# gyoge0/sub_volume_renderer

Hardware: AMD Instinct MI355X
Metric: Mray-steps/sec (+ frames/sec) of the LMIP sub-volume march at 1920x1080, 3-LOD 1024^3 volume (higher is better)
Workload: dtype f32

## Files before the change

sub_volume_renderer_amd/csrc/march_kernel.hip:

```cpp
#include <stdlib.h>

#include <algorithm>
#include <type_traits>

#include "svr_internal.h"

namespace {

struct f3 { float x, y, z; };
struct f4 { float x, y, z, w; };

__device__ __forceinline__ f4 mat_vec(const float* m, float x, float y, float z, float w) {
    f4 r;
    r.x = ((m[0] * x + m[4] * y) + m[8]  * z) + m[12] * w;
    r.y = ((m[1] * x + m[5] * y) + m[9]  * z) + m[13] * w;
    r.z = ((m[2] * x + m[6] * y) + m[10] * z) + m[14] * w;
    r.w = ((m[3] * x + m[7] * y) + m[11] * z) + m[15] * w;
    return r;
}

__device__ __forceinline__ float dot3(f3 a, f3 b) { return (a.x * b.x + a.y * b.y) + a.z * b.z; }

__device__ __forceinline__ uint32_t wrap(uint32_t t, uint32_t wrap0, uint32_t ring) {
    uint32_t w = t + wrap0;
// ... 348 lines not shown
__device__ __forceinline__ float texel_value(float t) { return t; }
__device__ __forceinline__ float texel_value(uint32_t t) { return (float)t; }
__device__ __forceinline__ float texel_abs(float t) { return fabsf(t); }
__device__ __forceinline__ uint32_t texel_abs(uint32_t t) { return t; }
__device__ __forceinline__ float texel_max(float a, float b) { return fmaxf(a, b); }
__device__ __forceinline__ uint32_t texel_max(uint32_t a, uint32_t b) { return max(a, b); }

template <int ESH>
__device__ __forceinline__ typename Texel<ESH>::type lds_texel(uint32_t a) {
#if defined(__HIP_DEVICE_COMPILE__)
    typedef __attribute__((address_space(3))) const uint8_t* p8_t;
    typedef __attribute__((address_space(3))) const uint16_t* p16_t;
    typedef __attribute__((address_space(3))) const float* p32_t;
    if constexpr (ESH == 2) return *(p32_t)a;
    else if constexpr (ESH == 1) return (uint32_t)*(p16_t)a;
    else return (uint32_t)*(p8_t)a;
#else
    (void)a;
    return typename Texel<ESH>::type();
#endif
}

template <int ESH>
__device__ __forceinline__ typename Texel<ESH>::type fetch_density(__amdgpu_buffer_rsrc_t rsrc, uint32_t off, uint32_t soff = 0u) {
    if constexpr (ESH == 2) return __builtin_bit_cast(float, __builtin_amdgcn_raw_buffer_load_b32(rsrc, (int)off, (int)soff, 0));
    else if constexpr (ESH == 1) return (uint32_t)(uint16_t)__builtin_amdgcn_raw_buffer_load_b16(rsrc, (int)off, (int)soff, 0);
    else return (uint32_t)(uint8_t)__builtin_amdgcn_raw_buffer_load_b8(rsrc, (int)off, (int)soff, 0);
}

__device__ __forceinline__ uint32_t mad24(uint32_t a, uint32_t b, uint32_t c) {
    uint32_t r;
    asm("v_mad_u32_u24 %0, %1, %2, %3" : "=v"(r) : "v"(a), "v"(b), "v"(c));
    return r;
}
template <int SH>
__device__ __forceinline__ uint32_t shl_add_c(uint32_t a, uint32_t c) {
    if (SH == 0) return a + c;
    uint32_t r;
    asm("v_lshl_add_u32 %0, %1, %2, %3" : "=v"(r) : "v"(a), "n"(SH), "v"(c));
    return r;
}

template <int ESH> struct TwinBlock { static constexpr int XB = ESH == 0 ? 3 : 2, YB = 2, ZB = ESH == 2 ? 1 : 2; };
struct TwinConsts { uint32_t row_w, inb_w, nbx32; };
template <int ESH>
__device__ __forceinline__ TwinConsts twin_consts(uint32_t Rx, uint32_t Ry) {
    typedef TwinBlock<ESH> B;
    TwinConsts c;
    c.row_w = 1u | (((Ry >> B::YB) * (4u >> B::ZB)) << 16);
    c.inb_w = (1u << (B::XB + ESH)) | ((1u << (B::XB + B::YB + ESH)) << 16);
    c.nbx32 = (Rx >> B::XB) * 32u;
    return c;
}
typedef unsigned short ushort2_t __attribute__((ext_vector_type(2)));
template <int ESH>
__device__ __forceinline__ uint32_t twin_offset_packed(uint32_t x, uint32_t yz, const TwinConsts& c, uint32_t KbS) {
    typedef TwinBlock<ESH> B;
    constexpr uint32_t xm = (1u << B::XB) - 1u, zm = (1u << B::ZB) - 1u, low = 3u | (zm << 16);
    const uint32_t xin = ESH == 0 ? ((x & xm) | KbS) : (((x & xm) << ESH) | KbS);
    const uint32_t inb = __builtin_amdgcn_udot2(__builtin_bit_cast(ushort2_t, yz & low), __builtin_bit_cast(ushort2_t, c.inb_w), xin, false);
    const uint32_t row4 = __builtin_amdgcn_udot2(__builtin_bit_cast(ushort2_t, yz & ~low), __builtin_bit_cast(ushort2_t, c.row_w), 0u, false);
    return __umul24(row4, c.nbx32) + (((x & ~xm) << (7 - B::XB)) + inb);
}
typedef short short2_t __attribute__((ext_vector_type(2)));
typedef float float2_t __attribute__((ext_vector_type(2)));

template <bool SC>
__device__ __forceinline__ float2_t coord_pair(float2_t iter, float s, float t, float ss) {
    if constexpr (SC) return iter * t + s;
    else return (iter * t + s) * ss;
}
template <bool SC>
__device__ __forceinline__ float coord_one(float iter, float s, float t, float ss) {
    if constexpr (SC) return iter * t + s;
    else return (iter * t + s) * ss;
}

struct Idx2 { uint32_t x0, y0, z0, x1, y1, z1; };
template <bool SC>
__device__ __forceinline__ Idx2 voxel_pair(float sx, float sy, float sz, float tx, float ty, float tz, float2_t iter,
                                           float ssx, float ssy, float ssz) {
    const float2_t cx = coord_pair<SC>(iter, sx, tx, ssx);
    const float2_t cy = coord_pair<SC>(iter, sy, ty, ssy);
    const float2_t cz = coord_pair<SC>(iter, sz, tz, ssz);
    Idx2 r;
    r.x0 = (uint32_t)(int)cx.x; r.x1 = (uint32_t)(int)cx.y;
    r.y0 = (uint32_t)(int)cy.x; r.y1 = (uint32_t)(int)cy.y;
    r.z0 = (uint32_t)(int)cz.x; r.z1 = (uint32_t)(int)cz.y;
    return r;
}

struct Idx2p { uint32_t x0, yz0, x1, yz1; };
template <bool SC>
__device__ __forceinline__ Idx2p voxel_pair_packed(float sx, float sy, float sz, float tx, float ty, float tz, float2_t iter,
                                                   float ssx, float ssy, float ssz) {
    const float2_t cx = coord_pair<SC>(iter, sx, tx, ssx);
    const float2_t cy = coord_pair<SC>(iter, sy, ty, ssy);
    const float2_t cz = coord_pair<SC>(iter, sz, tz, ssz);
    Idx2p r;
    r.x0 = (uint32_t)(int)cx.x; r.x1 = (uint32_t)(int)cx.y;
    r.yz0 = (uint32_t)(int)cy.x; r.yz1 = (uint32_t)(int)cy.y;
    asm("v_cvt_i32_f32_sdwa %0, %1 dst_sel:WORD_1 dst_unused:UNUSED_PRESERVE src0_sel:DWORD" : "+v"(r.yz0) : "v"(cz.x));
    asm("v_cvt_i32_f32_sdwa %0, %1 dst_sel:WORD_1 dst_unused:UNUSED_PRESERVE src0_sel:DWORD" : "+v"(r.yz1) : "v"(cz.y));
    return r;
}
__device__ __forceinline__ uint32_t dot2_u16(uint32_t a, uint32_t b, uint32_t c) {
    uint32_t r;
    asm("v_dot2_u32_u16 %0, %1, %2, %3" : "=v"(r) : "v"(a), "s"(b), "v"(c));
    return r;
}
template <typename T> __device__ __forceinline__ T undefined_value() { T v; asm volatile("" : "=v"(v)); return v; }

__device__ __forceinline__ void wave_min3_max3(int& a, int& b, int& c, int& d, int& e, int& f) {
#define SVR_STEP6(ctrl)                              \
    "v_min_i32_dpp %0, %0, %0 " ctrl "\n"            \
    "v_min_i32_dpp %1, %1, %1 " ctrl "\n"            \
    "v_min_i32_dpp %2, %2, %2 " ctrl "\n"            \
    "v_max_i32_dpp %3, %3, %3 " ctrl "\n"            \
    "v_max_i32_dpp %4, %4, %4 " ctrl "\n"            \
    "v_max_i32_dpp %5, %5, %5 " ctrl "\n"
    asm volatile("s_nop 1\n"
                 SVR_STEP6("quad_perm:[1,0,3,2] row_mask:0xf bank_mask:0xf")
                 SVR_STEP6("quad_perm:[2,3,0,1] row_mask:0xf bank_mask:0xf")
                 SVR_STEP6("row_half_mirror row_mask:0xf bank_mask:0xf")
                 SVR_STEP6("row_mirror row_mask:0xf bank_mask:0xf")
                 SVR_STEP6("row_bcast:15 row_mask:0xa bank_mask:0xf")
                 SVR_STEP6("row_bcast:31 row_mask:0xc bank_mask:0xf")
                 "s_nop 0"
                 : "+v"(a), "+v"(b), "+v"(c), "+v"(d), "+v"(e), "+v"(f));
#undef SVR_STEP6
    a = __builtin_amdgcn_readlane(a, 63); b = __builtin_amdgcn_readlane(b, 63); c = __builtin_amdgcn_readlane(c, 63);
    d = __builtin_amdgcn_readlane(d, 63); e = __builtin_amdgcn_readlane(e, 63); f = __builtin_amdgcn_readlane(f, 63);
}

template <bool MAX>
__device__ __forceinline__ int wave_reduce(int v) {
#define SVR_STEP1(ctrl) "s_nop 1\n" "v_min_i32_dpp %0, %0, %0 " ctrl "\n"
#define SVR_STEP1X(ctrl) "s_nop 1\n" "v_max_i32_dpp %0, %0, %0 " ctrl "\n"
    if (MAX)
        asm volatile(SVR_STEP1X("quad_perm:[1,0,3,2] row_mask:0xf bank_mask:0xf")
                     SVR_STEP1X("quad_perm:[2,3,0,1] row_mask:0xf bank_mask:0xf")
                     SVR_STEP1X("row_half_mirror row_mask:0xf bank_mask:0xf")
                     SVR_STEP1X("row_mirror row_mask:0xf bank_mask:0xf")
                     SVR_STEP1X("row_bcast:15 row_mask:0xa bank_mask:0xf")
                     SVR_STEP1X("row_bcast:31 row_mask:0xc bank_mask:0xf")
                     "s_nop 0" : "+v"(v));
    else
        asm volatile(SVR_STEP1("quad_perm:[1,0,3,2] row_mask:0xf bank_mask:0xf")
                     SVR_STEP1("quad_perm:[2,3,0,1] row_mask:0xf bank_mask:0xf")
                     SVR_STEP1("row_half_mirror row_mask:0xf bank_mask:0xf")
                     SVR_STEP1("row_mirror row_mask:0xf bank_mask:0xf")
                     SVR_STEP1("row_bcast:15 row_mask:0xa bank_mask:0xf")
                     SVR_STEP1("row_bcast:31 row_mask:0xc bank_mask:0xf")
                     "s_nop 0" : "+v"(v));
#undef SVR_STEP1
#undef SVR_STEP1X
    return __builtin_amdgcn_readlane(v, 63);
}

struct LodK {
    uint32_t ring[3];
    float    scale[3];
    int32_t  addw[3];
    uint32_t rx4, base_bytes;
    float    ss[3];
    int32_t  slab;
    const void* rbase;
    uint32_t rbytes;
    uint32_t nparts, zsplit, part_bytes, rbytes_last;
    uint32_t twin;
};
__device__ __forceinline__ LodK load_lod(kparams_t p, int l) {
    LodK k;
#pragma unroll
    for (int a = 0; a < 3; ++a) {
        k.ring[a] = p->lod[l].ring[a]; k.scale[a] = p->lod[l].scale[a]; k.addw[a] = p->lod[l].addw[a]; k.ss[a] = p->lod[l].ss[a];
    }
    k.rx4 = p->lod[l].rx4; k.base_bytes = p->lod[l].base_bytes; k.slab = p->lod[l].slab;
    k.rbase = p->lod[l].rbase; k.rbytes = p->lod[l].rbytes;
    k.nparts = p->lod[l].nparts; k.zsplit = p->lod[l].zsplit; k.part_bytes = p->lod[l].part_bytes; k.rbytes_last = p->lod[l].rbytes_last;
    k.twin = p->lod[l].twin;
    return k;
}

struct LodEvents {
    int a, b;
    int cx, cy, cz;
};


template <int NL, int U, bool COUNT, int ESH, bool BIG, bool WAVG = false, bool SCALED = false>
__global__ __launch_bounds__(256) __attribute__((amdgpu_waves_per_eu(SCALED && !COUNT ? 5 : 1))) void march_span(const MarchParams P) {
    static_assert(!(SCALED && WAVG), "the weighted-average reducer reads the unscaled step");
    extern __shared__ __attribute__((aligned(16))) uint8_t lds_all[];
    const int nblocks = P.tiles_x * P.tiles_y;
    const int tb = P.tile_order ? (int)P.tile_order[blockIdx.x] : xcd_remap((int)blockIdx.x, nblocks);
    const int tile_x = tb % P.tiles_x, tile_y = tb / P.tiles_x;
    const int wave = __builtin_amdgcn_readfirstlane((int)(threadIdx.x >> 6)), lane = threadIdx.x & 63;
    const int lw = P.tile_log2w, wl = P.block_waves_log2;
    const int c0 = ((tile_x << wl) + (wave & wl)) << lw, r0 = ((tile_y << wl) + (wave >> 1)) << (6 - lw);
    int lc = lane & ((1 << lw) - 1), lr = lane >> lw;
    {
        const float pcx = (float)(P.frame.x0 + c0) + 0.5f * (float)(1 << lw);
        const float pcy = (float)(P.frame.y0 + (r0 / P.frame.band_h) * P.frame.band_pitch + (r0 % P.frame.band_h)) +
                          0.5f * (float)(64 >> lw);
        const float ncx = 2.0f * pcx / (float)P.frame.frame_w - 1.0f;
        const float ncy = 1.0f - 2.0f * pcy / (float)P.frame.frame_h;
        const float dx = (P.xdir[0] - ncx * P.xdir[3]) * (float)P.frame.frame_w;
        const float dy = (P.xdir[1] - ncy * P.xdir[3]) * (float)P.frame.frame_h;
        if (P.orient && fabsf(dy) > fabsf(dx)) { lr = lane & ((64 >> lw) - 1); lc = lane >> (6 - lw); }
    }
    const int c = c0 + lc;
    const int r = r0 + lr;
    const bool inside = c < P.frame.out_w && r < P.frame.out_h;
    const size_t o = (size_t)r * (size_t)P.frame.out_w + (size_t)c;
    const int x = P.frame.x0 + c;
    const int y = P.frame.y0 + (r / P.frame.band_h) * P.frame.band_pitch + (r % P.frame.band_h);

    unsigned long long t_acc[16] = { 0, 0, 0, 0, 0, 0, 0, 0, 0, 0, 0, 0, 0, 0, 0, 0 };
    unsigned long long t_last = COUNT ? __builtin_amdgcn_s_memtime() : 0ull;
    auto lap = [&](int k) {
        if (COUNT) {
            const unsigned long long t = __builtin_amdgcn_s_memtime();
            t_acc[k] += t - t_last;
            t_last = t;
        }
    };

    Ray Rs;
    Rs.nsteps = 0; Rs.start = { 0.f, 0.f, 0.f }; Rs.step = { 0.f, 0.f, 0.f };
    const bool frag = inside && (x < P.frame.frame_w && y < P.frame.frame_h) && setup_ray(P, x, y, Rs);
    const int nsteps = frag ? Rs.nsteps : 0;
    float Rsx = frag ? Rs.start.x : 0.f, Rsy = frag ? Rs.start.y : 0.f, Rsz = frag ? Rs.start.z : 0.f;
    float Rtx = frag ? Rs.step.x : 0.f, Rty = frag ? Rs.step.y : 0.f, Rtz = frag ? Rs.step.z : 0.f;

    float d0[3], d1[3];
    {
        const float lastf = (float)(nsteps - 1);
        d0[0] = (Rsx + 0.0f * Rtx) * P.size[0];  d1[0] = (Rsx + lastf * Rtx) * P.size[0];
        d0[1] = (Rsy + 0.0f * Rty) * P.size[1];  d1[1] = (Rsy + lastf * Rty) * P.size[1];
        d0[2] = (Rsz + 0.0f * Rtz) * P.size[2];  d1[2] = (Rsz + lastf * Rtz) * P.size[2];
    }
    LodEvents ev[NL];
#pragma unroll
    for (int l = 0; l < NL; ++l) {
        const LodParams& L = P.lod[l];
        int a = 0, b = nsteps, cr[3] = { 0, 0, 0 };
        if (L.shape[0] == 0 || L.shape[1] == 0 || L.shape[2] == 0) {
            ev[l].a = 0; ev[l].b = 0; ev[l].cx = 0; ev[l].cy = 0; ev[l].cz = 0;
            continue;
        }
#pragma unroll
        for (int ax = 0; ax < 3; ++ax) {
            const float st = ax == 0 ? Rsx : (ax == 1 ? Rsy : Rsz);
            const float sp = ax == 0 ? Rtx : (ax == 1 ? Rty : Rtz);
            const bool inc = sp > 0.0f;
            const int v0 = (int)(d0[ax] * L.scale[ax]), v1 = (int)(d1[ax] * L.scale[ax]);
            auto cross = [&](int T) {
                const bool p0 = inc ? v0 >= T : v0 < T;
                const bool p1 = inc ? v1 >= T : v1 < T;
                int j = p0 ? 0 : nsteps;
                const bool need = !p0 && p1;
                if (__builtin_amdgcn_ballot_w64(need) != 0) {
                    const int js = first_cross(nsteps, st, sp, P.size[ax], L.scale[ax], T, need);
                    j = need ? js : j;
                }
                return j;
            };
            const int lo = L.off[ax], hi = L.off[ax] + (int)L.shape[ax];
            const int jlo = cross(lo);
            const int jhi = cross(hi);
            int en = inc ? jlo : jhi, ex = inc ? jhi : jlo;
            if (!(sp > 0.0f) && !(sp < 0.0f)) {
                en = 0; ex = (lo <= v0 && v0 < hi) ? nsteps : 0;
            }
            a = max(a, en); b = min(b, ex);
            if (L.wrap0[ax] + L.shape[ax] > L.ring[ax])
                cr[ax] = cross((int)L.ring[ax] - L.addw[ax]);
            else
                cr[ax] = inc ? nsteps : 0;
        }
        if (a >= b || L.shape[0] == 0) { a = 0; b = 0; }
        ev[l].a = a; ev[l].b = b; ev[l].cx = cr[0]; ev[l].cy = cr[1]; ev[l].cz = cr[2];
    }

    __amdgpu_buffer_rsrc_t rsrc_all = __builtin_amdgcn_make_buffer_rsrc(
        const_cast<void*>(P.density_all), 0, (int)P.density_all_bytes, 0x00020000);

#ifdef SVR_EXPERIMENTS
    const int dbg_nowait = P.dbg_nowait, brick_pow2 = P.brick_pow2;
#else
    constexpr int dbg_nowait = 0, brick_pow2 = 0;
#endif
    bool found = false, finished = (dbg_nowait & 2) != 0;
    float local_max = 0.f, samp = 0.f;
    int hit_i = 0, since = 0;
    uint32_t steps = 0;

    typedef typename Texel<ESH>::type texel_t;
    texel_t thr_raw;
    if constexpr (ESH != 2) thr_raw = P.lmip_threshold_raw; else thr_raw = P.lmip_threshold;
    const bool mip_like = (P.skip_flags & 2) != 0;
    float den = 0.f;
    auto lmip_batch = [&](const texel_t (&sv)[U], int nb, bool live, bool tail) {
        if constexpr (WAVG) {
            const float steplen = sqrtf((Rtx * Rtx + Rty * Rty) + Rtz * Rtz);
            const float k = fresh_params(P)->weight_falloff;
#pragma unroll
            for (int u = 0; u < U; ++u) {
                const bool act = live && !finished && (!tail || (nb + u) < nsteps);
                const float tw = 1.0f - k * ((float)(nb + u) * steplen);
                const bool go = act && tw > 0.0f;
                finished = finished || (act && !go);
                if (COUNT) steps += go ? 1u : 0u;
                const float val = texel_value(sv[u]);
                const float w = tw * tw;
                const float contribution = w * fabsf(val);
                const float num1 = samp + w * val, den1 = den + w;
                samp = go ? num1 : samp;
                den = go ? den1 : den;
                const bool take = go && contribution > local_max;
                local_max = take ? contribution : local_max;
                hit_i = take ? (nb + u) : hit_i;
            }
            return;
        }
        texel_t m;
        if constexpr (ESH != 2) m = 0u; else m = -1.0f;
        const texel_t neutral = m;
#pragma unroll
        for (int u = 0; u < U; ++u) m = texel_max(m, (tail && (nb + u) >= nsteps) ? neutral : texel_abs(sv[u]));
        bool need;
        if (mip_like) need = live && (found ? texel_value(m) > local_max : m >= thr_raw);
        else need = live && (found || m >= thr_raw);
        if (__builtin_amdgcn_ballot_w64(need) != 0) {
#pragma unroll
            for (int u = 0; u < U; ++u) {
                const bool act = live && !finished && (!tail || (nb + u) < nsteps);
                const float val = texel_value(sv[u]);
                const float inten = fabsf(val);
                if (COUNT) steps += act ? 1u : 0u;
                const bool was_found = found;
                const bool first_hit = act && !was_found && inten >= P.lmip_threshold;
                const bool tracking = act && was_found;
                since += tracking ? 1 : 0;
                const bool take = first_hit || (tracking && inten > local_max);
                local_max = take ? inten : local_max;
                samp = take ? val : samp;
                hit_i = take ? (nb + u) : hit_i;
                found = found || first_hit;
                const bool brk = tracking && (since >= P.lmip_max_samples || inten < local_max * P.lmip_fall_off);
                finished = finished || brk;
            }
        } else if (COUNT) {
            steps += live ? (uint32_t)(tail ? (min(nb + U, nsteps) - nb) : U) : 0u;
        }
    };

    int code = NL, E = 0;
    uint32_t Kc = 0xFFFFFFFFu;
    uint32_t Kb = 0u;
    int zth = 0;

    int brick_mode = 0;
    bool many_lines = false;
    if (P.brick) {
        const float pf = (float)min(max(nsteps - 1, 0), 256);
        const int qx = (int)((Rsx + pf * Rtx) * P.size[0]) >> (7 - ESH);
        const int qy = (int)((Rsy + pf * Rty) * P.size[1]);
        const int qz = (int)((Rsz + pf * Rtz) * P.size[2]);
        const int key = frag ? ((qz * 4099 + qy) * 64 + (qx & 63)) : -1 - lane;
        const int k0 = __builtin_amdgcn_update_dpp(key, key, 0x00, 0xF, 0xF, false);
        const int k1 = __builtin_amdgcn_update_dpp(key, key, 0x55, 0xF, 0xF, false);
        const int k2 = __builtin_amdgcn_update_dpp(key, key, 0xAA, 0xF, 0xF, false);
        const int q = lane & 3;
        const bool fresh = frag && (q == 0 || (key != k0 && (q == 1 || (key != k1 && (q == 2 || key != k2)))));
        const int lines = __builtin_popcountll(__builtin_amdgcn_ballot_w64(fresh));
        const int quads = __builtin_popcountll(__builtin_amdgcn_ballot_w64(frag && q == 0)) + 1;
        const bool use_brick = P.brick >= 2 || lines * 16 > P.brick_lines * quads;
        brick_mode = use_brick ? 1 + P.slab_long : 0;
        many_lines = use_brick;
    }
    const int wave_lds = wave * P.brick_bytes;

    int c_general = 0, c_direct = 0, c_brick = 0, c_slabs = 0, c_runs = 0, c_zero = 0, c_skip = 0;
    int n = 0;
    lap(0);
    while (true) {
        const bool alive = !finished && n < nsteps;
        const unsigned long long alive_mask = __builtin_amdgcn_ballot_w64(alive);
        if (alive_mask == 0) break;

        if (__builtin_amdgcn_ballot_w64(alive && n >= E) != 0) {
            const kparams_t Pr = fresh_params(P);
            if (alive && n >= E) {
                code = NL; E = nsteps; Kc = 0xFFFFFFFFu;
                bool settled = false;
#pragma unroll
                for (int l = 0; l < NL; ++l) {
                    const bool in = !settled && n >= ev[l].a && n < ev[l].b;
                    if (in) {
                        const LodK L = load_lod(Pr, l);
                        code = l;
                        E = min(E, ev[l].b);
                        const bool px = (n >= ev[l].cx) == (Rtx > 0.0f);
                        const bool py = (n >= ev[l].cy) == (Rty > 0.0f);
                        const bool pz = (n >= ev[l].cz) == (Rtz > 0.0f);
                        const uint32_t kx = (uint32_t)L.addw[0] - (px ? L.ring[0] : 0u);
                        const uint32_t ky = (uint32_t)L.addw[1] - (py ? L.ring[1] : 0u);
                        const uint32_t kz = (uint32_t)L.addw[2] - (pz ? L.ring[2] : 0u);
                        Kc = (kz * L.ring[1] + ky) * L.rx4 + (kx << ESH) + L.base_bytes;
                        if (many_lines && L.twin) {
                            typedef TwinBlock<ESH> B;
                            Kb = (uint32_t)(((int)kz >> B::ZB) * (int)(L.ring[1] >> B::YB) + ((int)ky >> B::YB)) * (L.ring[0] >> B::XB) +
                                 (uint32_t)((int)kx >> B::XB);
                        }
                        if constexpr (BIG) zth = (int)L.zsplit - (int)kz;
                        if (ev[l].cx > n) E = min(E, ev[l].cx);
                        if (ev[l].cy > n) E = min(E, ev[l].cy);
                        if (ev[l].cz > n) E = min(E, ev[l].cz);
                    } else if (!settled && ev[l].a > n) {
                        E = min(E, ev[l].a);
                    }
                    settled = settled || in;
                }
            }
        }

        const int first = __builtin_amdgcn_readlane(code, (int)__builtin_ctzll(alive_mask));
        int lane_run = (code == first) ? ((E == nsteps ? E - n + U - 1 : E - n) / U) : 0;
        if (first < NL && !fresh_params(P)->lod_pow2[first < NL ? first : 0]) lane_run = alive ? 0 : lane_run;
        if (!alive) lane_run = 0x3fffffff;
        int run = wave_reduce<false>(lane_run);
        if (COUNT) ++c_runs;
        lap(1);

        if (run <= 0) {
            if (COUNT) ++c_general;
            const kparams_t Pg = fresh_params(P);
            texel_t s[U];
            const float basef = (float)n;
            if constexpr (!BIG) {
                uint32_t off[U];
#pragma unroll
                for (int u = 0; u < U; ++u) {
                    off[u] = 0xFFFFFFFFu;
                    const float iter = basef + (float)u;
                    const float dx = (Rsx + iter * Rtx) * Pg->size[0];
                    const float dy = (Rsy + iter * Rty) * Pg->size[1];
                    const float dz = (Rsz + iter * Rtz) * Pg->size[2];
                    bool done = !alive || (n + u) >= nsteps;
#pragma unroll
                    for (int l = 0; l < NL; ++l) {
                        const bool sel = !done && (n + u) >= ev[l].a && (n + u) < ev[l].b;
                        if (__builtin_amdgcn_ballot_w64(sel) != 0) {
                            const uint32_t ofs = lod_offset_wrapped<ESH>(load_lod(Pg, l), dx, dy, dz);
                            off[u] = sel ? ofs : off[u];
                        }
                        done = done || sel;
                    }
                }
#pragma unroll
                for (int u = 0; u < U; ++u) s[u] = fetch_density<ESH>(rsrc_all, off[u]);
            } else {
#pragma unroll
                for (int u = 0; u < U; ++u) {
                    const float iter = basef + (float)u;
                    const float dx = (Rsx + iter * Rtx) * Pg->size[0];
                    const float dy = (Rsy + iter * Rty) * Pg->size[1];
                    const float dz = (Rsz + iter * Rtz) * Pg->size[2];
                    bool done = !alive || (n + u) >= nsteps;
                    texel_t acc = 0;
#pragma unroll
                    for (int l = 0; l < NL; ++l) {
                        const bool sel = !done && (n + u) >= ev[l].a && (n + u) < ev[l].b;
                        if (__builtin_amdgcn_ballot_w64(sel) != 0) {
                            const LodK Lg = load_lod(Pg, l);
                            uint32_t part;
                            const uint32_t ofs = lod_offset_wrapped_split<ESH>(Lg, dx, dy, dz, part);
                            for (unsigned long long todo = __builtin_amdgcn_ballot_w64(sel); todo != 0ull;) {
                                const uint32_t p = (uint32_t)__builtin_amdgcn_readlane((int)part, (int)__builtin_ctzll(todo));
                                const bool mine = sel && part == p;
                                const texel_t t = fetch_density<ESH>(part_rsrc(Lg, p), mine ? ofs : 0xFFFFFFFFu);
                                acc = mine ? t : acc;
                                todo &= ~__builtin_amdgcn_ballot_w64(mine);
                            }
                        }
                        done = done || sel;
                    }
                    s[u] = acc;
                }
            }
            lmip_batch(s, n, alive, true);
            n += U;
            lap(2);
            continue;
        }

        if (first == NL) {
            texel_t s[U];
#pragma unroll
            for (int u = 0; u < U; ++u) s[u] = 0;
            for (; run > 0; --run) {
                if (COUNT) ++c_zero;
                const bool lv = alive && !finished && n < nsteps;
                if (__builtin_amdgcn_ballot_w64(lv && n + U > nsteps) != 0) lmip_batch(s, n, lv, true);
                else lmip_batch(s, n, lv, false);
                n += U;
                if (__builtin_amdgcn_ballot_w64(alive && !finished && n < nsteps) == 0) break;
            }
            continue;
        }

        {
            const LodK L = load_lod(fresh_params(P), first);
            const float ssx = L.ss[0], ssy = L.ss[1], ssz = L.ss[2];
            if constexpr (SCALED) { Rsx *= ssx; Rsy *= ssy; Rsz *= ssz; Rtx *= ssx; Rty *= ssy; Rtz *= ssz; }
            __amdgpu_buffer_rsrc_t rsrc = rsrc_all;
            if constexpr (BIG) rsrc = __builtin_amdgcn_make_buffer_rsrc(const_cast<void*>(L.rbase), 0, (int)L.rbytes, 0x00020000);
            const bool ring_split = BIG && L.nparts > 1u;
            const bool use_twin = many_lines && L.twin == 1u;

            int held = 0;
            do {
            run += held; held = 0;
            if (P.cells_all_bytes != 0u) {
                const kparams_t Ps = fresh_params(P);
                const int sb = Ps->lod[first].skip_batches;
                if (sb > 0 && run >= 4 * sb) {
                    const float reach = (float)(8 * sb);
                    const uint32_t cs = (uint32_t)Ps->lod[first].cshift;
                    const float vx = SCALED ? Rtx : Rtx * ssx, vy = SCALED ? Rty : Rty * ssy, vz = SCALED ? Rtz : Rtz * ssz;
                    const bool slow = fmaxf(fmaxf(fabsf(vx), fabsf(vy)), fabsf(vz)) * reach <=
                                      (float)(1u << cs) - 0.5f;
                    __amdgpu_buffer_rsrc_t crsrc = __builtin_amdgcn_make_buffer_rsrc(
                        const_cast<void*>(Ps->cells_all), 0, (int)Ps->cells_all_bytes, 0x00020000);
                    const uint32_t cbase = Ps->lod[first].cell_base;
                    const uint32_t cdx = Ps->lod[first].cdim[0], cdy = Ps->lod[first].cdim[1], cdz = Ps->lod[first].cdim[2];
                    bool vetoed = false, tracking_only = false;
                    uint32_t c0x, c0y, c0z;
                    {
                        const float i0 = fminf((float)n, (float)(nsteps - 1));
                        c0x = ((uint32_t)(int)coord_one<SCALED>(i0, Rsx, Rtx, ssx) + (uint32_t)L.addw[0]) >> cs;
                        c0y = ((uint32_t)(int)coord_one<SCALED>(i0, Rsy, Rty, ssy) + (uint32_t)L.addw[1]) >> cs;
                        c0z = ((uint32_t)(int)coord_one<SCALED>(i0, Rsz, Rtz, ssz) + (uint32_t)L.addw[2]) >> cs;
                    }
                    while (run >= 4 * sb) {
                        const bool live = alive && !finished && n < nsteps;
                        const float lastf = fminf((float)(nsteps - 1), (float)n + 4.0f * reach - (run > 4 * sb ? 0.0f : 1.0f));
                        uint32_t px[5], py[5], pz[5];
                        px[0] = c0x; py[0] = c0y; pz[0] = c0z;
#pragma unroll
                        for (int g = 1; g < 5; g += 2) {
                            const float i0 = (float)n + reach * (float)g;
                            const float2_t iter = { fminf(i0, lastf), fminf(i0 + reach, lastf) };
                            const Idx2 q = voxel_pair<SCALED>(Rsx, Rsy, Rsz, Rtx, Rty, Rtz, iter, ssx, ssy, ssz);
                            px[g] = (q.x0 + (uint32_t)L.addw[0]) >> cs; py[g] = (q.y0 + (uint32_t)L.addw[1]) >> cs; pz[g] = (q.z0 + (uint32_t)L.addw[2]) >> cs;
                            px[g + 1] = (q.x1 + (uint32_t)L.addw[0]) >> cs; py[g + 1] = (q.y1 + (uint32_t)L.addw[1]) >> cs;
                            pz[g + 1] = (q.z1 + (uint32_t)L.addw[2]) >> cs;
                        }
                        c0x = px[4]; c0y = py[4]; c0z = pz[4];
                        texel_t v[4];
#pragma unroll
                        for (int g = 0; g < 4; ++g) {
                            uint32_t bx = min(px[g], px[g + 1]), by = min(py[g], py[g + 1]), bz = min(pz[g], pz[g + 1]);
                            bx = min(bx, bx - cdx); by = min(by, by - cdy); bz = min(bz, bz - cdz);
                            v[g] = fetch_density<ESH>(crsrc, (__umul24(__umul24(bz, cdy) + by, cdx) + bx) << ESH, cbase);
                        }
                        const texel_t m = texel_max(texel_max(texel_abs(v[0]), texel_abs(v[1])), texel_max(texel_abs(v[2]), texel_abs(v[3])));
                        const bool occupied = live && !found && (!slow || m >= thr_raw);
                        const bool following = live && found && (!mip_like || !slow || texel_value(m) > local_max);
                        const unsigned long long occ_mask = __builtin_amdgcn_ballot_w64(occupied);
                        if (occ_mask != 0 || __builtin_amdgcn_ballot_w64(following) != 0) {
                            vetoed = true;
                            tracking_only = occ_mask == 0;
                            break;
                        }
                        if (COUNT) { steps += live ? (uint32_t)(min(n + 32 * sb, nsteps) - n) : 0u; c_skip += 4 * sb; }
                        n += 32 * sb;
                        run -= 4 * sb;
                        if (__builtin_amdgcn_ballot_w64(alive && !finished && n < nsteps) == 0) { run = 0; break; }
                    }
                    if (vetoed) {
                        int cap = 4 * sb;
                        if (brick_mode && L.slab > 0 && !use_twin) cap = max(cap, (L.slab << (brick_mode - 1)) / U);
                        if (tracking_only && (P.skip_flags & 1) && !mip_like) cap = min(cap, 2);
                        if (run > cap) { held = run - cap; run = cap; }
                    }
                }
                lap(10);
            }

            {
                while (brick_mode && L.slab > 0 && !use_twin && run >= (L.slab << (brick_mode - 1)) / U) {
                    const int slab = L.slab << (brick_mode - 1);
                    const bool live = alive && !finished && n < nsteps;
                    const float2_t it = { (float)n, (float)min(n + slab - 1, nsteps - 1) };
                    const float2_t ex = coord_pair<SCALED>(it, Rsx, Rtx, ssx);
                    const float2_t ey = coord_pair<SCALED>(it, Rsy, Rty, ssy);
                    const float2_t ez = coord_pair<SCALED>(it, Rsz, Rtz, ssz);
                    const int big = 0x7fffffff;
                    int lx = live ? min((int)ex.x, (int)ex.y) : big, hx = live ? max((int)ex.x, (int)ex.y) : -big;
                    int ly = live ? min((int)ey.x, (int)ey.y) : big, hy = live ? max((int)ey.x, (int)ey.y) : -big;
                    int lz = live ? min((int)ez.x, (int)ez.y) : big, hz = live ? max((int)ez.x, (int)ez.y) : -big;
#if defined(SVR_EXPERIMENTS) && defined(SVR_EXP_NO_BOX_REDUCE)
                    lx = __builtin_amdgcn_readfirstlane(lx); ly = __builtin_amdgcn_readfirstlane(ly); lz = __builtin_amdgcn_readfirstlane(lz);
                    hx = lx + 12; hy = ly + 10; hz = lz + 10;
#else
                    wave_min3_max3(lx, ly, lz, hx, hy, hz);
#endif
                    if (COUNT) ++c_slabs;
                    lap(8);
                    if (lx == big) { run = 0; break; }
                    constexpr int GSH = 4 - ESH;
                    const int gx0 = lx - ((lx + L.addw[0]) & ((1 << GSH) - 1));
                    const int ngx = ((hx - gx0) >> GSH) + 1;
                    const int ny = hy - ly + 1, nz = hz - lz + 1;
                    const int gp = brick_pow2 ? (ngx <= 1 ? 1 : 1 << (32 - __builtin_clz(ngx - 1))) : (ngx | 1);
                    const int pz = brick_pow2 ? ny * gp : ((ny * gp) | 1);
                    if (ny >= 512 || pz * nz * 16 > P.brick_bytes) {
                        if (brick_mode > 1) { --brick_mode; continue; }
                        brick_mode = 0; break;
                    }
                    const float rgp = __builtin_amdgcn_rcpf((float)gp);
                    const int rows_per = (int)(64.5f * rgp);
                    const int ly_lane = (int)(((float)lane + 0.5f) * rgp);
                    const int g_lane = lane - ly_lane * gp;
                    uint32_t wx = (uint32_t)(gx0 + (g_lane << GSH) + L.addw[0]);
                    wx = min(wx, wx - L.ring[0]);
                    wx <<= ESH;
                    const uint32_t plane_bytes = (uint32_t)(pz << 4);
                    const uint32_t zpitch = L.ring[1] * L.rx4;
                    lap(9);
#if defined(SVR_EXPERIMENTS) && defined(SVR_EXP_NO_BRICK_LOADS)
                    if (false)
#endif
                    for (int yc = 0; yc < ny; yc += rows_per) {
                        const int yy = yc + ly_lane;
                        uint32_t wy = (uint32_t)(ly + yy + L.addw[1]);
                        wy = min(wy, wy - L.ring[1]);
                        const uint32_t lane_src = mad24(wy, L.rx4, L.base_bytes + wx);
                        const uint32_t lds_chunk = (uint32_t)wave_lds + (uint32_t)((yc * gp) << 4);
                        if (yy < ny && g_lane < ngx && ly_lane < rows_per) {
                            for (int zz = 0; zz < nz; ++zz) {
                                uint32_t wz = (uint32_t)(lz + zz + L.addw[2]);
                                wz = min(wz, wz - L.ring[2]);
                                if (BIG && ring_split) {
                                    uint32_t p = 0u;
                                    while (p + 1u < L.nparts && wz >= (p + 1u) * L.zsplit) ++p;
                                    __builtin_amdgcn_raw_ptr_buffer_load_lds(
                                        part_rsrc(L, p), (__attribute__((address_space(3))) void*)(lds_all + lds_chunk + zz * plane_bytes),
                                        16, (int)(lane_src + (wz - p * L.zsplit) * zpitch), 0, 0, 0);
                                } else
                                __builtin_amdgcn_raw_ptr_buffer_load_lds(
                                    rsrc, (__attribute__((address_space(3))) void*)(lds_all + lds_chunk + zz * plane_bytes),
                                    16, (int)(lane_src + wz * zpitch), 0, 0, 0);
                            }
                        }
                    }
                    const uint32_t lds_base = (uint32_t)reinterpret_cast<uintptr_t>((__attribute__((address_space(3))) uint8_t*)lds_all);
                    const uint32_t bk = lds_base + (uint32_t)wave_lds - (uint32_t)(((lz * pz + ly * gp) << 4) + (gx0 << ESH));
                    lap(3);
                    if (!(dbg_nowait & 1)) asm volatile("s_waitcnt vmcnt(0)" ::: "memory");
                    lap(4);
                    const uint32_t kyz = (uint32_t)(gp << 4) | ((uint32_t)(pz << 4) << 16);
                    const bool slab_tail = __builtin_amdgcn_ballot_w64(live && n + slab > nsteps) != 0;
                    for (int k = 0; k < slab / U; ++k) {
                        texel_t s[U];
                        float2_t iter = { (float)n, (float)n + 1.0f };
#pragma unroll
                        for (int u = 0; u < U; u += 2) {
                            const Idx2p v = voxel_pair_packed<SCALED>(Rsx, Rsy, Rsz, Rtx, Rty, Rtz, iter, ssx, ssy, ssz);
                            iter += 2.0f;
                            const uint32_t a0 = dot2_u16(v.yz0, kyz, shl_add_c<ESH>(v.x0, bk));
                            const uint32_t a1 = dot2_u16(v.yz1, kyz, shl_add_c<ESH>(v.x1, bk));
                            s[u] = lds_texel<ESH>(a0);
                            s[u + 1] = lds_texel<ESH>(a1);
                        }
                        if constexpr (ESH != 2 && U == 8)
                            asm("" : "+v"(s[0]), "+v"(s[1]), "+v"(s[2]), "+v"(s[3]), "+v"(s[4]), "+v"(s[5]), "+v"(s[6]), "+v"(s[7]));
                        {
                            const bool lv = alive && !finished && n < nsteps;
                            if (slab_tail && __builtin_amdgcn_ballot_w64(lv && n + U > nsteps) != 0) lmip_batch(s, n, lv, true);
                            else lmip_batch(s, n, lv, false);
                        }
                        n += U;
                        if (COUNT) ++c_brick;
                    }
                    run -= slab / U;
                    lap(5);
                    asm volatile("" ::: "memory");
                }
            }

            __amdgpu_buffer_rsrc_t rsrc_twin = rsrc;
            const void* twin_base = nullptr;
            auto direct_batches = [&](auto from_twin) {
            constexpr bool TW = decltype(from_twin)::value;
            for (; run > 0; --run) {
                const bool live = alive && !finished && n < nsteps;
                if (__builtin_amdgcn_ballot_w64(live) == 0) break;
                if (COUNT) { ++c_direct; if (TW) t_acc[15] += 1ull; }
                texel_t s[U];
                uint32_t off[U];
                float2_t iter = { (float)n, (float)n + 1.0f };
                if constexpr (TW) {
                    const TwinConsts tc = twin_consts<ESH>(L.ring[0], L.ring[1]);
                    const uint32_t KbS = Kb << 7;
#pragma unroll
                    for (int u = 0; u < U; u += 2) {
                        const Idx2p v = voxel_pair_packed<SCALED>(Rsx, Rsy, Rsz, Rtx, Rty, Rtz, iter, ssx, ssy, ssz);
                        iter += 2.0f;
                        off[u] = twin_offset_packed<ESH>(v.x0, v.yz0, tc, KbS);
                        off[u + 1] = twin_offset_packed<ESH>(v.x1, v.yz1, tc, KbS);
                    }
                } else {
#pragma unroll
                for (int u = 0; u < U; u += 2) {
                    const Idx2 v = voxel_pair<SCALED>(Rsx, Rsy, Rsz, Rtx, Rty, Rtz, iter, ssx, ssy, ssz);
                    iter += 2.0f;
                    off[u] = mad24(mad24(v.z0, L.ring[1], v.y0), L.rx4, shl_add_c<ESH>(v.x0, Kc));
                    off[u + 1] = mad24(mad24(v.z1, L.ring[1], v.y1), L.rx4, shl_add_c<ESH>(v.x1, Kc));
                }
                }
#pragma unroll
                for (int u = 0; u < U; ++u) s[u] = undefined_value<texel_t>();
                if (BIG && ring_split) {
                    auto part_of = [&](int icz) {
                        uint32_t q = 0u;
                        for (uint32_t k = 1; k < L.nparts; ++k) q += icz >= zth + (int)((k - 1u) * L.zsplit) ? 1u : 0u;
                        return q;
                    };
                    const float2_t ends = { (float)n, (float)min(n + U - 1, nsteps - 1) };
                    const float2_t ez2 = coord_pair<SCALED>(ends, Rsz, Rtz, ssz);
                    const uint32_t pa = part_of((int)ez2.x), pb = part_of((int)ez2.y);
                    const uint32_t p0 = (uint32_t)__builtin_amdgcn_readlane((int)pa, (int)__builtin_ctzll(__builtin_amdgcn_ballot_w64(live)));
                    if (__builtin_amdgcn_ballot_w64(live && (pa != p0 || pb != p0)) == 0) {
                        const __amdgpu_buffer_rsrc_t rp = part_rsrc(L, p0, TW ? twin_base : L.rbase);
                        const uint32_t sub = p0 * L.part_bytes;
#pragma unroll
                        for (int u = 0; u < U; ++u) s[u] = fetch_density<ESH>(rp, live ? off[u] - sub : 0xFFFFFFFFu);
                    } else {
                    float2_t it2 = { (float)n, (float)n + 1.0f };
#pragma unroll
                    for (int u = 0; u < U; u += 2) {
                        const float2_t cz = coord_pair<SCALED>(it2, Rsz, Rtz, ssz);
                        it2 += 2.0f;
#pragma unroll
                        for (int h = 0; h < 2; ++h) {
                            const int icz = h ? (int)cz.y : (int)cz.x;
                            uint32_t part = 0u;
                            for (uint32_t k = 1; k < L.nparts; ++k) part += icz >= zth + (int)((k - 1u) * L.zsplit) ? 1u : 0u;
                            const uint32_t rel = off[u + h] - part * L.part_bytes;
                            texel_t a = 0;
                            for (unsigned long long todo = __builtin_amdgcn_ballot_w64(live); todo != 0ull;) {
                                const uint32_t p = (uint32_t)__builtin_amdgcn_readlane((int)part, (int)__builtin_ctzll(todo));
                                const bool mine = live && part == p;
                                const texel_t t = fetch_density<ESH>(part_rsrc(L, p, TW ? twin_base : L.rbase), mine ? rel : 0xFFFFFFFFu);
                                a = mine ? t : a;
                                todo &= ~__builtin_amdgcn_ballot_w64(mine);
                            }
                            s[u + h] = a;
                        }
                    }
                    }
                } else
                if (live) {
#pragma unroll
                    for (int u = 0; u < U; ++u) s[u] = fetch_density<ESH>(TW ? rsrc_twin : rsrc, off[u]);
                }
                if (__builtin_amdgcn_ballot_w64(live && n + U > nsteps) != 0) lmip_batch(s, n, live, true);
                else lmip_batch(s, n, live, false);
                n += U;
            }
            };
            if (use_twin || (many_lines && L.twin == 2u && (brick_mode == 0 || L.slab <= 0))) {
                const kparams_t Pt = fresh_params(P);
                twin_base = Pt->lod[first].twin_rbase;
                rsrc_twin = __builtin_amdgcn_make_buffer_rsrc(const_cast<void*>(twin_base), 0, (int)Pt->lod[first].twin_rbytes, 0x00020000);
                direct_batches(std::true_type{});
            } else {
                direct_batches(std::false_type{});
            }
            } while (held > 0 && __builtin_amdgcn_ballot_w64(alive && !finished && n < nsteps) != 0);
            if constexpr (SCALED) {
                const kparams_t Pu = fresh_params(P);
                const float ux = Pu->lod[first].rss[0], uy = Pu->lod[first].rss[1], uz = Pu->lod[first].rss[2];
                Rsx *= ux; Rsy *= uy; Rsz *= uz; Rtx *= ux; Rty *= uy; Rtz *= uz;
            }
            lap(6);
        }
    }

    if (COUNT && P.dbg && lane == 0) {
        atomicAdd(P.dbg + 0, (uint32_t)c_general); atomicAdd(P.dbg + 1, (uint32_t)c_direct);
        atomicAdd(P.dbg + 2, (uint32_t)c_brick);   atomicAdd(P.dbg + 3, (uint32_t)c_slabs);
        atomicAdd(P.dbg + 4, (uint32_t)c_runs);    atomicAdd(P.dbg + 5, (uint32_t)c_zero);
        atomicAdd(P.dbg + 6, 1u);                  atomicAdd(P.dbg + 7, (uint32_t)c_skip);
    }
    Hit h;
    h.found = found; h.sample = samp; h.steps = steps;
    if constexpr (WAVG) { h.found = local_max > 0.0f; h.sample = h.found ? samp / den : 0.0f; }
    const float hit_f = (float)hit_i;
    h.offset = { hit_f * Rtx, hit_f * Rty, hit_f * Rtz };
    h.coord = { Rsx + h.offset.x, Rsy + h.offset.y, Rsz + h.offset.z };
    if (inside) {
#if defined(__HIP_DEVICE_COMPILE__)
        const MarchParams* Pk = (const MarchParams*)__builtin_amdgcn_kernarg_segment_ptr();
        asm volatile("" : "+s"(Pk));
#else
        const MarchParams* Pk = &P;
#endif
        shade_and_store<NL>(*Pk, o, frag, h);
        if (COUNT && Pk->steps) Pk->steps[o] = h.steps;
    }
    if (COUNT && P.dbg) {
        lap(7);
        if (lane == 0) {
            unsigned long long* t_out = reinterpret_cast<unsigned long long*>(P.dbg + 8);
#pragma unroll
            for (int k = 0; k < 16; ++k) atomicAdd(t_out + k, t_acc[k]);
        }
    }
}

template <int NL>
hipError_t launch_nl(const MarchParams& p, int kind, hipStream_t stream) {
    const int nblocks = p.tiles_x * p.tiles_y;
    if (nblocks <= 0) return hipSuccess;
    const bool simple = kind == 1 || !p.span_ok;
    const bool wavg = p.render_mode == SVR_MODE_WEIGHTED_AVERAGE;
    if (wavg && (simple || p.per_lod_rsrc)) {
        if (p.steps) hipLaunchKernelGGL((march_wavg<NL, true>), dim3(nblocks), dim3(256), 0, stream, p);
        else         hipLaunchKernelGGL((march_wavg<NL, false>), dim3(nblocks), dim3(256), 0, stream, p);
    } else if (simple) {
        if (p.steps) hipLaunchKernelGGL((march_simple<NL, true>), dim3(nblocks), dim3(256), 0, stream, p);
        else         hipLaunchKernelGGL((march_simple<NL, false>), dim3(nblocks), dim3(256), 0, stream, p);
    } else {
        const int threads = 64 << (2 * p.block_waves_log2);
        const size_t lds = (size_t)p.brick_bytes * (threads / 64);
#define SVR_LAUNCH_SPAN_SC(ESH_, SC_)                                                                                              \
    do {                                                                                                                           \
        if (p.per_lod_rsrc) {                                                                                                      \
            if (p.steps) hipLaunchKernelGGL((march_span<NL, 8, true, ESH_, true>), dim3(nblocks), dim3(threads), lds, stream, p);   \
            else         hipLaunchKernelGGL((march_span<NL, 8, false, ESH_, true>), dim3(nblocks), dim3(threads), lds, stream, p);  \
        } else {                                                                                                                   \
            if (p.steps) hipLaunchKernelGGL((march_span<NL, 8, true, ESH_, false, false, SC_>), dim3(nblocks), dim3(threads), lds, stream, p);  \
            else         hipLaunchKernelGGL((march_span<NL, 8, false, ESH_, false, false, SC_>), dim3(nblocks), dim3(threads), lds, stream, p); \
        }                                                                                                                          \
    } while (0)
#define SVR_LAUNCH_SPAN(ESH_)                                                                                              \
    do {                                                                                                                   \
        if (p.ss_pow2 && !p.per_lod_rsrc) SVR_LAUNCH_SPAN_SC(ESH_, true);                                                  \
        else           SVR_LAUNCH_SPAN_SC(ESH_, false);                                                                    \
    } while (0)
#define SVR_LAUNCH_WAVG(ESH_)                                                                                              \
    do {                                                                                                                   \
        if (p.steps) hipLaunchKernelGGL((march_span<NL, 8, true, ESH_, false, true>), dim3(nblocks), dim3(threads), lds, stream, p);   \
        else         hipLaunchKernelGGL((march_span<NL, 8, false, ESH_, false, true>), dim3(nblocks), dim3(threads), lds, stream, p);  \
    } while (0)
        if (wavg) {
            if (p.density_esh == 0) SVR_LAUNCH_WAVG(0);
            else if (p.density_esh == 1) SVR_LAUNCH_WAVG(1);
            else SVR_LAUNCH_WAVG(2);
        }
        else if (p.density_esh == 0) SVR_LAUNCH_SPAN(0);
        else if (p.density_esh == 1) SVR_LAUNCH_SPAN(1);
        else SVR_LAUNCH_SPAN(2);
#undef SVR_LAUNCH_WAVG
#undef SVR_LAUNCH_SPAN
#undef SVR_LAUNCH_SPAN_SC
    }
    return hipGetLastError();
}

}

#ifndef SVR_NL
#error "compile with -DSVR_NL=<number of LODs>"
#endif
#define SVR_CAT2(a, b) a##b
#define SVR_CAT(a, b) SVR_CAT2(a, b)
hipError_t SVR_CAT(svr_launch_march_nl, SVR_NL)(const MarchParams& p, int kind, hipStream_t stream) {
    return launch_nl<SVR_NL>(p, kind, stream);
}
```

Baseline: 1.980 million.

## Split march runs into tail-free interior batches and recheck liveness only after hits

The wave-reduced run length now also encodes how many batches stay fully inside nsteps for every lane. Batches in that interior run skip the per-batch tail ballot and the tail masking. The live predicate is recomputed only when lmip_batch actually fired, and the iteration counter is carried forward instead of being rebuilt each batch. The zero-run, brick-slab and direct paths all use this, which removes per-batch ballots and compares from the hot loop but makes the run bookkeeping more complex and more fragile at the run boundaries.

```diff
diff --git a/sub_volume_renderer_amd/csrc/march_kernel.hip b/sub_volume_renderer_amd/csrc/march_kernel.hip
--- a/sub_volume_renderer_amd/csrc/march_kernel.hip
+++ b/sub_volume_renderer_amd/csrc/march_kernel.hip
@@ -674,7 +674,7 @@
     if constexpr (ESH != 2) thr_raw = P.lmip_threshold_raw; else thr_raw = P.lmip_threshold;
     const bool mip_like = (P.skip_flags & 2) != 0;
     float den = 0.f;
-    auto lmip_batch = [&](const texel_t (&sv)[U], int nb, bool live, bool tail) {
+    auto lmip_batch = [&](const texel_t (&sv)[U], int nb, bool live, bool tail) -> bool {
         if constexpr (WAVG) {
             const float steplen = sqrtf((Rtx * Rtx + Rty * Rty) + Rtz * Rtz);
             const float k = fresh_params(P)->weight_falloff;
@@ -695,7 +695,7 @@
                 local_max = take ? contribution : local_max;
                 hit_i = take ? (nb + u) : hit_i;
             }
-            return;
+            return true;
         }
         texel_t m;
         if constexpr (ESH != 2) m = 0u; else m = -1.0f;
@@ -705,7 +705,8 @@
         bool need;
         if (mip_like) need = live && (found ? texel_value(m) > local_max : m >= thr_raw);
         else need = live && (found || m >= thr_raw);
-        if (__builtin_amdgcn_ballot_w64(need) != 0) {
+        const bool fired = __builtin_amdgcn_ballot_w64(need) != 0;
+        if (fired) {
 #pragma unroll
             for (int u = 0; u < U; ++u) {
                 const bool act = live && !finished && (!tail || (nb + u) < nsteps);
@@ -727,6 +728,7 @@
         } else if (COUNT) {
             steps += live ? (uint32_t)(tail ? (min(nb + U, nsteps) - nb) : U) : 0u;
         }
+        return fired;
     };
 
     int code = NL, E = 0;
@@ -800,10 +802,12 @@
         }
 
         const int first = __builtin_amdgcn_readlane(code, (int)__builtin_ctzll(alive_mask));
-        int lane_run = (code == first) ? ((E == nsteps ? E - n + U - 1 : E - n) / U) : 0;
+        int lane_run = (code == first) ? ((E == nsteps ? E - n + U - 1 : E - n) / U + (E - n) / U) : 0;
         if (first < NL && !fresh_params(P)->lod_pow2[first < NL ? first : 0]) lane_run = alive ? 0 : lane_run;
         if (!alive) lane_run = 0x3fffffff;
-        int run = wave_reduce<false>(lane_run);
+        const int run_key = wave_reduce<false>(lane_run);
+        int run = (run_key + 1) >> 1;
+        const int nfull = n + (run_key >> 1) * U;
         if (COUNT) ++c_runs;
         lap(1);
 
@@ -873,11 +877,22 @@
             texel_t s[U];
 #pragma unroll
             for (int u = 0; u < U; ++u) s[u] = 0;
+            if (run > 0 && n + U <= nfull) {
+                bool lv = alive && !finished;
+                do {
+                    if (COUNT) ++c_zero;
+                    const bool fired = lmip_batch(s, n, lv, false);
+                    n += U; --run;
+                    if (fired) {
+                        lv = alive && !finished;
+                        if (__builtin_amdgcn_ballot_w64(lv) == 0) run = 0;
+                    }
+                } while (run > 0 && n + U <= nfull);
+            }
             for (; run > 0; --run) {
                 if (COUNT) ++c_zero;
                 const bool lv = alive && !finished && n < nsteps;
-                if (__builtin_amdgcn_ballot_w64(lv && n + U > nsteps) != 0) lmip_batch(s, n, lv, true);
-                else lmip_batch(s, n, lv, false);
+                lmip_batch(s, n, lv, true);
                 n += U;
                 if (__builtin_amdgcn_ballot_w64(alive && !finished && n < nsteps) == 0) break;
             }
@@ -1036,10 +1051,10 @@
                     if (!(dbg_nowait & 1)) asm volatile("s_waitcnt vmcnt(0)" ::: "memory");
                     lap(4);
                     const uint32_t kyz = (uint32_t)(gp << 4) | ((uint32_t)(pz << 4) << 16);
-                    const bool slab_tail = __builtin_amdgcn_ballot_w64(live && n + slab > nsteps) != 0;
+                    float2_t iter = { it.x, it.x + 1.0f };
+                    bool lv = live;
                     for (int k = 0; k < slab / U; ++k) {
                         texel_t s[U];
-                        float2_t iter = { (float)n, (float)n + 1.0f };
 #pragma unroll
                         for (int u = 0; u < U; u += 2) {
                             const Idx2p v = voxel_pair_packed<SCALED>(Rsx, Rsy, Rsz, Rtx, Rty, Rtz, iter, ssx, ssy, ssz);
@@ -1052,9 +1067,10 @@
                         if constexpr (ESH != 2 && U == 8)
                             asm("" : "+v"(s[0]), "+v"(s[1]), "+v"(s[2]), "+v"(s[3]), "+v"(s[4]), "+v"(s[5]), "+v"(s[6]), "+v"(s[7]));
                         {
-                            const bool lv = alive && !finished && n < nsteps;
-                            if (slab_tail && __builtin_amdgcn_ballot_w64(lv && n + U > nsteps) != 0) lmip_batch(s, n, lv, true);
-                            else lmip_batch(s, n, lv, false);
+                            bool fired;
+                            if (n + U <= nfull) fired = lmip_batch(s, n, lv, false);
+                            else { lv = alive && !finished && n < nsteps; fired = lmip_batch(s, n, lv, true); }
+                            if (fired) lv = alive && !finished && n + U < nsteps;
                         }
                         n += U;
                         if (COUNT) ++c_brick;
@@ -1069,13 +1085,10 @@
             const void* twin_base = nullptr;
             auto direct_batches = [&](auto from_twin) {
             constexpr bool TW = decltype(from_twin)::value;
-            for (; run > 0; --run) {
-                const bool live = alive && !finished && n < nsteps;
-                if (__builtin_amdgcn_ballot_w64(live) == 0) break;
+            auto batch = [&](auto interior, const bool live, float2_t& iter) -> bool {
                 if (COUNT) { ++c_direct; if (TW) t_acc[15] += 1ull; }
                 texel_t s[U];
                 uint32_t off[U];
-                float2_t iter = { (float)n, (float)n + 1.0f };
                 if constexpr (TW) {
                     const TwinConsts tc = twin_consts<ESH>(L.ring[0], L.ring[1]);
                     const uint32_t KbS = Kb << 7;
@@ -1141,9 +1154,28 @@
 #pragma unroll
                     for (int u = 0; u < U; ++u) s[u] = fetch_density<ESH>(TW ? rsrc_twin : rsrc, off[u]);
                 }
-                if (__builtin_amdgcn_ballot_w64(live && n + U > nsteps) != 0) lmip_batch(s, n, live, true);
-                else lmip_batch(s, n, live, false);
+                const bool fired = lmip_batch(s, n, live, !decltype(interior)::value);
                 n += U;
+                return fired;
+            };
+            if (run > 0 && n + U <= nfull) {
+                bool live = alive && !finished;
+                if (__builtin_amdgcn_ballot_w64(live) == 0) return;
+                float2_t iter = { (float)n, (float)n + 1.0f };
+                do {
+                    const bool fired = batch(std::true_type{}, live, iter);
+                    --run;
+                    if (fired) {
+                        live = alive && !finished;
+                        if (__builtin_amdgcn_ballot_w64(live) == 0) return;
+                    }
+                } while (run > 0 && n + U <= nfull);
+            }
+            for (; run > 0; --run) {
+                const bool live = alive && !finished && n < nsteps;
+                if (__builtin_amdgcn_ballot_w64(live) == 0) break;
+                float2_t iter = { (float)n, (float)n + 1.0f };
+                batch(std::false_type{}, live, iter);
             }
             };
             if (use_twin || (many_lines && L.twin == 2u && (brick_mode == 0 || L.slab <= 0))) {
```

Result: no change. 1.984 million (median of 2 runs) (+0.2%).
